# apache/tez

Measured on NVIDIA H100. Metric: sorted KV GB/s (16B key / 64B val), higher is better.
Workload: dtype u8

## Files before the change

tez_b200/csrc/common.cuh:

```cuda
#pragma once
#include <cuda_runtime.h>
#include <stdint.h>
#include <stdio.h>

#include <stdexcept>
#include <string>

namespace tezgpu {

struct Error : public std::runtime_error {
  int code;
  Error(int c, const std::string &m) : std::runtime_error(m), code(c) {}
};

#define TG_CUDA(expr)                                                                                   \
  do {                                                                                                  \
    cudaError_t _e = (expr);                                                                            \
    if (_e != cudaSuccess) {                                                                            \
      throw ::tezgpu::Error(_e == cudaErrorMemoryAllocation ? -3 : -2,                                  \
                            std::string(#expr) + ": " + cudaGetErrorString(_e) + " (" + __FILE__ + ":" + \
                                std::to_string(__LINE__) + ")");                                        \
    }                                                                                                   \
  } while (0)

#define TG_CHECK(cond, code, msg)                      \
  do {                                                 \
    if (!(cond)) throw ::tezgpu::Error((code), (msg)); \
  } while (0)

static inline uint64_t div_up(uint64_t a, uint64_t b) { return (a + b - 1) / b; }
static inline uint64_t align_up(uint64_t a, uint64_t b) { return div_up(a, b) * b; }

enum { CMP_BYTES = 0, CMP_TEXT = 1, CMP_BYTESWRITABLE = 2, CMP_INT = 3, CMP_LONG = 4 };

__host__ __device__ __forceinline__ int vint_decode_size(uint8_t first) {
  int v = (int)(int8_t)first;
  if (v >= -112) return 1;
  if (v < -120) return -119 - v;
  return -111 - v;
}
__host__ __device__ __forceinline__ int vint_size_u32(uint32_t v) {
  if (v <= 127) return 1;
  if (v < (1u << 8)) return 2;
  if (v < (1u << 16)) return 3;
  if (v < (1u << 24)) return 4;
  return 5;
}
__host__ __device__ __forceinline__ uint8_t vint_byte_u32(uint32_t v, int b) {
  int sz = vint_size_u32(v);
  if (sz == 1) return (uint8_t)v;
  if (b == 0) return (uint8_t)(-112 - (sz - 1));
  int shift = (sz - 1 - b) * 8;
  return (uint8_t)(v >> shift);
}

__device__ __forceinline__ uint32_t key_content_skip(int cmp, const uint8_t *key, uint32_t klen) {
  if (klen == 0) return 0;
  if (cmp == CMP_TEXT) {
    uint32_t s = (uint32_t)vint_decode_size(key[0]);
    return s < klen ? s : klen;
  }
  if (cmp == CMP_BYTESWRITABLE) return klen < 4 ? klen : 4;
  return 0;
}

__device__ __forceinline__ uint32_t norm_byte(int cmp, const uint8_t *content, uint32_t i) {
  uint32_t b = content[i];
  if (i == 0 && (cmp == CMP_INT || cmp == CMP_LONG)) b ^= 0x80u;
  return b;
}

__device__ __forceinline__ int32_t hash_bytes_dev(const uint8_t *p, uint32_t n) {
  uint32_t h = 1;
  for (uint32_t i = 0; i < n; i++) h = 31u * h + (uint32_t)(int32_t)(int8_t)p[i];
  return (int32_t)h;
}

__device__ __forceinline__ int32_t key_hash_dev(int cmp, const uint8_t *key, uint32_t klen) {
  if (cmp == CMP_INT && klen >= 4)
    return (int32_t)(((uint32_t)key[0] << 24) | ((uint32_t)key[1] << 16) | ((uint32_t)key[2] << 8) | key[3]);
  if (cmp == CMP_LONG && klen >= 8) {
    uint64_t v = 0;
    for (int i = 0; i < 8; i++) v = (v << 8) | key[i];
    return (int32_t)(uint32_t)(v ^ (v >> 32));
  }
  uint32_t s = key_content_skip(cmp, key, klen);
  return hash_bytes_dev(key + s, klen - s);
}

__device__ __forceinline__ uint32_t lanemask_lt() {
  uint32_t m;
  asm("mov.u32 %0, %%lanemask_lt;" : "=r"(m));
  return m;
}

__device__ __forceinline__ uint32_t ld_volatile_u32(const uint32_t *p) {
  uint32_t v;
  asm volatile("ld.volatile.global.u32 %0, [%1];" : "=r"(v) : "l"(p) : "memory");
  return v;
}
__device__ __forceinline__ void st_volatile_u32(uint32_t *p, uint32_t v) {
  asm volatile("st.volatile.global.u32 [%0], %1;" ::"l"(p), "r"(v) : "memory");
}

__device__ __forceinline__ uint64_t ld_volatile_u64(const uint64_t *p) {
  uint64_t v;
  asm volatile("ld.volatile.global.u64 %0, [%1];" : "=l"(v) : "l"(p) : "memory");
  return v;
}
__device__ __forceinline__ void st_volatile_u64(uint64_t *p, uint64_t v) {
  asm volatile("st.volatile.global.u64 [%0], %1;" ::"l"(p), "l"(v) : "memory");
}

}
```

tez_b200/csrc/radix_sort.cuh:

```cuda
#pragma once
#include "common.cuh"

#ifndef TEZGPU_RADIX_THREADS32
#define TEZGPU_RADIX_THREADS32 512
#endif
#ifndef TEZGPU_RADIX_IPT32
#define TEZGPU_RADIX_IPT32 16
#endif
#ifndef TEZGPU_RADIX_LOOKBACK
#define TEZGPU_RADIX_LOOKBACK 8
#endif
#ifndef TEZGPU_RANK_MODE
#define TEZGPU_RANK_MODE 2
#endif

namespace tezgpu {

constexpr int RADIX_BITS = 8;
constexpr int RADIX = 1 << RADIX_BITS;
constexpr uint32_t STATE_FLAG_LOCAL = 1u << 30;
constexpr uint32_t STATE_FLAG_INCL = 2u << 30;
constexpr uint32_t STATE_VALUE_MASK = (1u << 30) - 1;
constexpr uint32_t RADIX_MAX_N = (1u << 30) - 1;

template <typename KeyT>
__device__ __forceinline__ uint32_t radix_digit(KeyT k, int shift) {
  return (uint32_t)(k >> shift) & (RADIX - 1);
}

template <typename KeyT, int NPASS>
__global__ void __launch_bounds__(512) k_radix_hist(const KeyT *__restrict__ keys, uint32_t n, int begin_bit,
                                                    uint32_t *__restrict__ hist ) {
  __shared__ uint32_t s_hist[NPASS * RADIX];
  for (int i = threadIdx.x; i < NPASS * RADIX; i += blockDim.x) s_hist[i] = 0;
  __syncthreads();
  uint32_t stride = gridDim.x * blockDim.x;
  for (uint32_t i = blockIdx.x * blockDim.x + threadIdx.x; i < n; i += stride) {
    KeyT k = keys[i];
#pragma unroll
    for (int p = 0; p < NPASS; p++) atomicAdd(&s_hist[p * RADIX + radix_digit(k, begin_bit + p * RADIX_BITS)], 1u);
  }
  __syncthreads();
  for (int i = threadIdx.x; i < NPASS * RADIX; i += blockDim.x) {
    uint32_t c = s_hist[i];
    if (c) atomicAdd(&hist[i], c);
  }
}

__global__ void __launch_bounds__(RADIX) k_radix_scan_hist(uint32_t *__restrict__ hist, int npass, uint32_t n,
                                                          uint32_t *__restrict__ trivial) {
  __shared__ uint32_t s_warp[RADIX / 32];
  const int tid = threadIdx.x, lane = tid & 31, warp = tid >> 5;
  for (int p = 0; p < npass; p++) {
    uint32_t c = hist[p * RADIX + tid];
    uint32_t incl = c;
#pragma unroll
    for (int o = 1; o < 32; o <<= 1) {
      uint32_t t = __shfl_up_sync(0xffffffffu, incl, o);
      if (lane >= o) incl += t;
    }
    if (lane == 31) s_warp[warp] = incl;
    __syncthreads();
    uint32_t base = 0;
    for (int w = 0; w < warp; w++) base += s_warp[w];
    hist[p * RADIX + tid] = base + incl - c;
    uint32_t any = __syncthreads_or(c == n && n > 0);
    if (tid == 0 && trivial) trivial[p] = any ? 1u : 0u;
    __syncthreads();
  }
}

template <typename KeyT, int THREADS, int IPT>
struct OnesweepCfg {
  static constexpr int NWARPS = THREADS / 32;
  static constexpr int TILE = THREADS * IPT;
  static constexpr size_t SMEM = (size_t)TILE * (sizeof(KeyT) + sizeof(uint32_t)) + (size_t)NWARPS * RADIX * 4 +
                                 2 * RADIX * 4 + 64 + (TEZGPU_RANK_MODE == 2 ? (size_t)NWARPS * RADIX * 4 : 0);
};

template <typename KeyT, int THREADS, int IPT, bool VALS_IOTA>
__global__ void __launch_bounds__(THREADS, 1024 / THREADS)
    k_onesweep_pass(const KeyT *__restrict__ keys_in, KeyT *__restrict__ keys_out, const uint32_t *__restrict__ vals_in,
                    uint32_t *__restrict__ vals_out, uint32_t n, int shift, const uint32_t *__restrict__ hist_base,
                    uint32_t *tile_state, uint32_t *tile_counter) {
  using Cfg = OnesweepCfg<KeyT, THREADS, IPT>;
  constexpr int NWARPS = Cfg::NWARPS;
  constexpr int TILE = Cfg::TILE;
  static_assert(THREADS >= RADIX, "one thread per digit for the look-back");

  extern __shared__ __align__(16) uint8_t smem_raw[];
  KeyT *s_keys = reinterpret_cast<KeyT *>(smem_raw);
  uint32_t *s_vals = reinterpret_cast<uint32_t *>(smem_raw + (size_t)TILE * sizeof(KeyT));
  uint32_t *s_wcnt = s_vals + TILE;
  uint32_t *s_dstart = s_wcnt + NWARPS * RADIX;
  uint32_t *s_goff = s_dstart + RADIX;
  uint32_t *s_misc = s_goff + RADIX;
#if TEZGPU_RANK_MODE == 2
  uint32_t *s_wmask = s_misc + 16;
#endif

  const int tid = threadIdx.x, lane = tid & 31, warp = tid >> 5;

#ifdef TEZGPU_TICKET_ATOMIC
  if (tid == 0) s_misc[0] = atomicAdd(tile_counter, 1u);
#else
  if (tid == 0) s_misc[0] = blockIdx.x;
#endif
  for (int i = tid; i < NWARPS * RADIX; i += THREADS) s_wcnt[i] = 0;
#if TEZGPU_RANK_MODE == 2
  for (int i = tid; i < NWARPS * RADIX; i += THREADS) s_wmask[i] = 0;
#endif
  __syncthreads();
  const uint32_t tile = s_misc[0];
  const uint32_t tile_base = tile * (uint32_t)TILE;
  const uint32_t tile_n = min((uint32_t)TILE, n - tile_base);
  const uint32_t warp_base = (uint32_t)warp * 32u * IPT;

  KeyT key[IPT];
  uint32_t rnk[IPT];
#pragma unroll
  for (int j = 0; j < IPT; j++) {
    uint32_t li = warp_base + j * 32 + lane;
    key[j] = (li < tile_n) ? keys_in[tile_base + li] : (KeyT)0;
  }
  uint32_t *wc = s_wcnt + warp * RADIX;
  const uint32_t lt = lanemask_lt();
#pragma unroll
  for (int j = 0; j < IPT; j++) {
    uint32_t li = warp_base + j * 32 + lane;
    bool valid = li < tile_n;
    uint32_t d = radix_digit(key[j], shift);
    uint32_t peers;
#if TEZGPU_RANK_MODE == 0
    peers = __match_any_sync(0xffffffffu, valid ? d : (uint32_t)RADIX);
#elif TEZGPU_RANK_MODE == 2
    {
      uint32_t *wm = s_wmask + warp * RADIX;
      if (valid) atomicOr(&wm[d], 1u << lane);
      __syncwarp();
      peers = valid ? wm[d] : 0u;
      __syncwarp();
      if (valid) atomicAnd(&wm[d], ~(1u << lane));
    }
#else
    peers = __ballot_sync(0xffffffffu, valid);
    if (!valid) peers = ~peers;
#pragma unroll
    for (int b = 0; b < RADIX_BITS; b++) {
      const bool bit = (d >> b) & 1u;
      const uint32_t bm = __ballot_sync(0xffffffffu, bit);
      peers &= bit ? bm : ~bm;
    }
#endif
    uint32_t pre = 0;
    if (valid && (peers & lt) == 0) pre = atomicAdd(&wc[d], (uint32_t)__popc(peers));
    pre = __shfl_sync(0xffffffffu, pre, __ffs(peers) - 1);
    rnk[j] = pre + __popc(peers & lt);
  }
  __syncthreads();

  uint32_t count = 0;
  if (tid < RADIX) {
    uint32_t run = 0;
#pragma unroll
    for (int w = 0; w < NWARPS; w++) {
      uint32_t c = s_wcnt[w * RADIX + tid];
      s_wcnt[w * RADIX + tid] = run;
      run += c;
    }
    count = run;
    st_volatile_u32(&tile_state[(size_t)tile * RADIX + tid], (tile == 0 ? STATE_FLAG_INCL : STATE_FLAG_LOCAL) | count);
    uint32_t incl = count;
#pragma unroll
    for (int o = 1; o < 32; o <<= 1) {
      uint32_t t = __shfl_up_sync(0xffffffffu, incl, o);
      if (lane >= o) incl += t;
    }
    if (lane == 31) s_misc[1 + warp] = incl;
    s_dstart[tid] = incl - count;
  }
  __syncthreads();
  if (tid < RADIX) {
    uint32_t base = 0;
    for (int w = 0; w < warp; w++) base += s_misc[1 + w];
    s_dstart[tid] += base;
  }
  __syncthreads();

#pragma unroll
  for (int j = 0; j < IPT; j++) {
    uint32_t li = warp_base + j * 32 + lane;
    if (li < tile_n) {
      uint32_t d = radix_digit(key[j], shift);
      uint32_t slot = s_dstart[d] + wc[d] + rnk[j];
      s_keys[slot] = key[j];
      uint32_t v;
      if (VALS_IOTA) v = tile_base + li;
      else v = vals_in[tile_base + li];
      s_vals[slot] = v;
    }
  }

  if (tid < RADIX) {
    uint32_t excl = 0;
    if (tile > 0) {
      constexpr int LOOKBACK = TEZGPU_RADIX_LOOKBACK;
      int64_t t = (int64_t)tile - 1;
      bool done = false;
      while (!done) {
        uint32_t st[LOOKBACK];
#ifdef TEZGPU_RADIX_DEBUG
        if (tid == 0) atomicAdd(tile_counter + 7, 1u);
#endif
#pragma unroll
        for (int b = 0; b < LOOKBACK; b++)
          st[b] = (t - b >= 0) ? ld_volatile_u32(&tile_state[(size_t)(t - b) * RADIX + tid]) : STATE_FLAG_INCL;
#pragma unroll
        for (int b = 0; b < LOOKBACK; b++) {
          if (done) break;
          uint32_t flag = st[b] & ~STATE_VALUE_MASK;
          if (flag == 0) break;
          excl += st[b] & STATE_VALUE_MASK;
          t--;
          if (flag == STATE_FLAG_INCL) done = true;
        }
      }
      st_volatile_u32(&tile_state[(size_t)tile * RADIX + tid], STATE_FLAG_INCL | (excl + count));
    }
    s_goff[tid] = hist_base[tid] + excl - s_dstart[tid];
  }
  __syncthreads();

#pragma unroll
  for (int k = 0; k < IPT; k++) {
    uint32_t slot = (uint32_t)tid + k * THREADS;
    if (slot < tile_n) {
      KeyT kk = s_keys[slot];
      uint32_t dest = s_goff[radix_digit(kk, shift)] + slot;
      keys_out[dest] = kk;
      vals_out[dest] = s_vals[slot];
    }
  }
}

struct RadixWorkspace {
  uint32_t *hist = nullptr;
  uint32_t *trivial = nullptr;
  uint32_t *tile_state = nullptr;
  uint32_t *tile_counter = nullptr;
  size_t tile_state_words = 0;
};

template <typename KeyT>
struct RadixTuning {
  static constexpr int THREADS = sizeof(KeyT) == 4 ? TEZGPU_RADIX_THREADS32 : 512;
  static constexpr int IPT = sizeof(KeyT) == 4 ? TEZGPU_RADIX_IPT32 : 10;
};

template <typename KeyT>
static inline uint32_t radix_num_tiles(uint32_t n) {
  using T = RadixTuning<KeyT>;
  return (uint32_t)div_up(n, (uint64_t)T::THREADS * T::IPT);
}
template <typename KeyT>
static inline size_t radix_tile_state_words(uint32_t n, int npass) {
  return (size_t)radix_num_tiles<KeyT>(n) * RADIX * (size_t)npass;
}

template <typename KeyT>
static int radix_sort_passes(cudaStream_t st, const RadixWorkspace &ws, KeyT *keys_a, KeyT *keys_b, uint32_t *vals_a,
                             uint32_t *vals_b, uint32_t n, int begin_bit, int npass, uint32_t pass_mask,
                             bool first_vals_iota, int *launches) {
  using T = RadixTuning<KeyT>;
  using Cfg = OnesweepCfg<KeyT, T::THREADS, T::IPT>;
  static bool attr_set = false;
  if (!attr_set) {
    TG_CUDA(cudaFuncSetAttribute(k_onesweep_pass<KeyT, T::THREADS, T::IPT, false>,
                                 cudaFuncAttributeMaxDynamicSharedMemorySize, (int)Cfg::SMEM));
    TG_CUDA(cudaFuncSetAttribute(k_onesweep_pass<KeyT, T::THREADS, T::IPT, true>,
                                 cudaFuncAttributeMaxDynamicSharedMemorySize, (int)Cfg::SMEM));
    attr_set = true;
  }
  uint32_t ntiles = radix_num_tiles<KeyT>(n);
  TG_CHECK((size_t)ntiles * RADIX * (size_t)npass <= ws.tile_state_words, -1, "radix workspace too small");
  TG_CUDA(cudaMemsetAsync(ws.tile_state, 0, (size_t)ntiles * RADIX * (size_t)npass * 4, st));
  TG_CUDA(cudaMemsetAsync(ws.tile_counter, 0, 8 * 4, st));
  int done = 0;
  bool iota = first_vals_iota;
  for (int p = 0; p < npass; p++) {
    if (!((pass_mask >> p) & 1u)) continue;
    KeyT *kin = (done & 1) ? keys_b : keys_a, *kout = (done & 1) ? keys_a : keys_b;
    uint32_t *vin = (done & 1) ? vals_b : vals_a, *vout = (done & 1) ? vals_a : vals_b;
    uint32_t *state = ws.tile_state + (size_t)p * ntiles * RADIX;
    if (iota)
      k_onesweep_pass<KeyT, T::THREADS, T::IPT, true><<<ntiles, T::THREADS, Cfg::SMEM, st>>>(
          kin, kout, vin, vout, n, begin_bit + p * RADIX_BITS, ws.hist + p * RADIX, state, ws.tile_counter + p);
    else
      k_onesweep_pass<KeyT, T::THREADS, T::IPT, false><<<ntiles, T::THREADS, Cfg::SMEM, st>>>(
          kin, kout, vin, vout, n, begin_bit + p * RADIX_BITS, ws.hist + p * RADIX, state, ws.tile_counter + p);
    TG_CUDA(cudaGetLastError());
    if (launches) (*launches)++;
    iota = false;
    done++;
  }
  return done;
}

}
```

tez_b200/csrc/sorter.cuh:

```cuda
#pragma once
#include <stdlib.h>
#include <string.h>

#include <vector>

#include "../../include/tezgpu.h"
#include "device_util.h"
#ifndef TEZGPU_EMIT_ROUND_FILL_DEFAULT
#define TEZGPU_EMIT_ROUND_FILL_DEFAULT 0
#endif
#include "emit_pipe_u.cuh"
#include "emit_tma.cuh"
#include "emit_runs.cuh"
#include "sorter_kernels.cuh"

namespace tezgpu {

__global__ void k_store_to_host(uint32_t *__restrict__ dst0, const uint32_t *__restrict__ src0, uint32_t n0, uint32_t *__restrict__ dst1,
                                const uint32_t *__restrict__ src1, uint32_t n1, uint32_t *__restrict__ dst2,
                                const uint32_t *__restrict__ src2, uint32_t n2) {
  for (uint32_t i = threadIdx.x; i < n0; i += blockDim.x) dst0[i] = src0[i];
  for (uint32_t i = threadIdx.x; i < n1; i += blockDim.x) dst1[i] = src1[i];
  for (uint32_t i = threadIdx.x; i < n2; i += blockDim.x) dst2[i] = src2[i];
  __threadfence_system();
}
static inline void store_to_host(cudaStream_t st, void *d0, const void *s0, size_t b0, void *d1 = nullptr, const void *s1 = nullptr,
                                 size_t b1 = 0, void *d2 = nullptr, const void *s2 = nullptr, size_t b2 = 0) {
  k_store_to_host<<<1, 256, 0, st>>>((uint32_t *)d0, (const uint32_t *)s0, (uint32_t)(b0 / 4), (uint32_t *)d1, (const uint32_t *)s1,
                                     (uint32_t)(b1 / 4), (uint32_t *)d2, (const uint32_t *)s2, (uint32_t)(b2 / 4));
}


static inline int partition_bits(int P) {
  int b = 0;
  while ((1ll << b) < (long long)P) b++;
  return b;
}

struct DeviceConstants {
  CrcTables *d_crc = nullptr;
  static DeviceConstants &get(int device) {
    static DeviceConstants inst[64];
    DeviceConstants &d = inst[device & 63];
    if (!d.d_crc) {
      CrcTables *h = new CrcTables();
      crc_build_tables(*h, EMIT_CRC_STRIDE_WORDS);
      TG_CUDA(cudaMalloc((void **)&d.d_crc, sizeof(CrcTables)));
      TG_CUDA(cudaMemcpy(d.d_crc, h, sizeof(CrcTables), cudaMemcpyHostToDevice));
      delete h;
    }
    return d;
  }
};

struct FramingMismatch {};

class SortPipeline {
 public:
  tezgpu_conf conf;
  int pbits;
  cudaStream_t stream = nullptr;
  EventTimer timer;
  int num_sms = 132;

  DeviceBuffer keysA, keysB, valsA, valsB, same, blk, small, tile_state, sizes, rec_off;
  DeviceBuffer t_pos[2], t_gid[2], t_lidx[2], t_key64[2], t_val[2], t_state, t_ghead, t_gneq, sym_sets, sym_tab, rep_flags;
  DeviceBuffer seg_start, tile_start, part_start, d_index, seg_crc, tile_desc, tile_crc, tie_state;
  PinnedBuffer h_small;

  explicit SortPipeline(const tezgpu_conf &c) : conf(c) {
    TG_CHECK(c.num_partitions >= 1, TEZGPU_E_INVALID, "num_partitions must be >= 1");
    TG_CHECK(c.comparator >= TEZGPU_CMP_BYTES && c.comparator <= TEZGPU_CMP_LONG, TEZGPU_E_UNSUPPORTED,
             "comparator outside the device-supported set (BYTES, TEXT, BYTESWRITABLE, INT, LONG)");
    TG_CHECK(c.partitioner == TEZGPU_PART_GIVEN || c.partitioner == TEZGPU_PART_HASH, TEZGPU_E_UNSUPPORTED,
             "partitioner outside the device-supported set (GIVEN, HASH)");
    int ndev = 0;
    cudaError_t e = cudaGetDeviceCount(&ndev);
    if (e != cudaSuccess || ndev == 0) {
      cudaGetLastError();
      throw Error(TEZGPU_E_CUDA, "no CUDA device available (libtezgpu has no CPU fallback)");
    }
    TG_CHECK(c.device >= 0 && c.device < ndev, TEZGPU_E_INVALID, "bad device ordinal");
    TG_CUDA(cudaSetDevice(c.device));
    TG_CUDA(cudaStreamCreateWithFlags(&stream, cudaStreamNonBlocking));
    TG_CUDA(cudaDeviceGetAttribute(&num_sms, cudaDevAttrMultiProcessorCount, c.device));
    {
      const char *g = getenv("TEZGPU_L2_FETCH");
      int gran = g ? atoi(g) : 32;
      if (gran > 0 && cudaDeviceSetLimit(cudaLimitMaxL2FetchGranularity, (size_t)gran) != cudaSuccess) cudaGetLastError();
    }
    pbits = partition_bits(c.num_partitions);
    TG_CHECK(pbits <= 31, TEZGPU_E_INVALID, "too many partitions");
    h_small.ensure(4096);
    small.ensure(16384);
    DeviceConstants::get(c.device);
  }
  ~SortPipeline() {
    if (stream) cudaStreamDestroy(stream);
  }

  static uint64_t output_bound(uint64_t n, uint64_t kv_bytes, int P) { return kv_bytes + 12 * n + 10ull * P + 64; }

  uint32_t *d_hist() { return small.as<uint32_t>(); }
  uint32_t *d_trivial() { return small.as<uint32_t>() + 2048; }
  uint32_t *d_tile_counter() { return small.as<uint32_t>() + 2056; }
  int *d_error() { return reinterpret_cast<int *>(small.as<uint32_t>() + 2064); }
  uint32_t *d_large() { return small.as<uint32_t>() + 2065; }
  uint32_t *d_m() { return small.as<uint32_t>() + 2072; }
  unsigned long long *d_ties() { return reinterpret_cast<unsigned long long *>(small.as<uint32_t>() + 2074); }
  uint32_t *d_ticket() { return small.as<uint32_t>() + 2073; }
  unsigned long long *d_dups() { return reinterpret_cast<unsigned long long *>(small.as<uint32_t>() + 2066); }
  uint64_t *d_totals() { return reinterpret_cast<uint64_t *>(small.as<uint32_t>() + 2068); }

  struct SortState {
    Records rec;
    uint32_t *K = nullptr;
    uint32_t *order = nullptr;
    uint64_t dup_count = 0, tie_records = 0;
    int launches = 0;
    bool have_bounds = false, spec_layout = false;
    uint64_t spec_file_bytes = 0, spec_tiles = 0;
  } state;
  int merge_check_same = 1;
  bool merge_inputs_plain = false;
  uint32_t merge_max_runs = 0;
  static bool runs_emit_enabled() {
    static const bool on = getenv("TEZGPU_EMIT_RUNS") && atoi(getenv("TEZGPU_EMIT_RUNS")) != 0;
    return on;
  }

  EmitParams make_emit_params(const Records &rec, const uint32_t *order, int rle, bool merge_mode, uint8_t *d_out) {
    EmitParams e;
    memset(&e, 0, sizeof(e));
    e.rec = rec;
    e.order = order;
    e.same = same.as<uint8_t>();
    e.part_start = part_start.as<uint32_t>();
    e.seg_start = seg_start.as<uint64_t>();
    e.tile_start = tile_start.as<uint32_t>();
    e.out = d_out;
    e.seg_crc = seg_crc.as<uint32_t>();
    e.crc = DeviceConstants::get(conf.device).d_crc;
    e.rle = rle;
    e.send_empty = conf.send_empty_partition_details;
    e.unordered = conf.sorter_impl == TEZGPU_SORTER_UNORDERED;
    e.merge_mode = merge_mode ? 1 : 0;
    e.check_same = merge_check_same;
    e.P = conf.num_partitions;
    return e;
  }
  static bool pipe_unaligned_enabled() {
    static const bool on = !(getenv("TEZGPU_EMIT_PIPE_UNALIGNED") && atoi(getenv("TEZGPU_EMIT_PIPE_UNALIGNED")) == 0);
    return on;
  }
  void set_fixed_layout(EmitParams &e, const Records &rec) {
    int h = 0;
    for (int b = 0; b < vint_size_u32(rec.klen); b++) e.fixed_hdr[h++] = vint_byte_u32(rec.klen, b);
    for (int b = 0; b < vint_size_u32(rec.vlen); b++) e.fixed_hdr[h++] = vint_byte_u32(rec.vlen, b);
    e.fixed_hdr_len = h;
    e.rec_size = h + rec.klen + rec.vlen;
    e.recs_per_tile = std::max<uint32_t>(1, std::min<uint32_t>(EMIT_MAX_RECS, (FE_IMG_BYTES - 32) / e.rec_size));
    static const int round_fill = getenv("TEZGPU_EMIT_ROUND_FILL") ? atoi(getenv("TEZGPU_EMIT_ROUND_FILL")) : TEZGPU_EMIT_ROUND_FILL_DEFAULT;
    bool fill = round_fill != 0;
    const uint32_t stride = rec.klen + rec.vlen;
    const bool fast = stride >= 16 && stride % 16 == 0;
    const bool aligned = !rec.key_off && !rec.use_runs && (((uintptr_t)rec.kv & 15u) == 0);
    if (rec.use_runs && runs_emit_enabled() && emit_runs_fits(e.recs_per_tile, e.rec_size, merge_max_runs)) {
    } else if (fast && aligned && emit4_max_recs(e.rec_size) >= 1 && emit4_fits(emit4_max_recs(e.rec_size), stride / 16, e.rec_size)) {
      e.recs_per_tile = std::min<uint32_t>(e.recs_per_tile, emit4_max_recs(e.rec_size));
    } else if (pipe_unaligned_enabled()) {
      if (fast && !aligned && emit4u_max_recs(stride / 16) >= 32) {
        e.recs_per_tile = std::min<uint32_t>(e.recs_per_tile, emit4u_max_recs(stride / 16));
        fill = true;
      }
    }
    if (fill && e.recs_per_tile >= 32) {
      const uint32_t cap = e.recs_per_tile;
      uint32_t best = cap;
      double best_eff = 0;
      for (uint32_t r = cap; r >= cap - cap / 10; r--) {
        const uint64_t chunks = ((uint64_t)r * e.rec_size + 15 + 4 + 2 + 15) / 16;
        const uint64_t rounds = (chunks + FE_THREADS - 1) / FE_THREADS;
        const double eff = (double)r / (double)rounds;
        if (eff > best_eff) { best_eff = eff; best = r; }
      }
      e.recs_per_tile = best;
    }
    e.rec_off = nullptr;
  }

  void run(Records rec, uint8_t *d_out, uint64_t out_cap, uint64_t *out_len, int64_t *index, tezgpu_stats *stats) {
    sort_phase(rec);
    int rle;
    if (conf.rle_policy == TEZGPU_RLE_ON) rle = 1;
    else if (conf.rle_policy == TEZGPU_RLE_OFF) rle = 0;
    else rle = (conf.sorter_impl == 1) ? 0 : ((double)state.dup_count > 0.1 * (double)rec.n);
    if (conf.sorter_impl == TEZGPU_SORTER_UNORDERED) rle = 0;
    emit_phase(rle, false, d_out, out_cap, out_len, index, stats);
  }

  void sort_phase(Records rec) {
    TG_CUDA(cudaSetDevice(conf.device));
    const uint32_t n = rec.n;
    const int P = conf.num_partitions;
    TG_CHECK(n <= RADIX_MAX_N, TEZGPU_E_INVALID, "more than 2^30-1 records in one sort");
    rec.cmp = conf.comparator;
    rec.hash_partition = conf.partitioner == TEZGPU_PART_HASH;
    rec.num_partitions = P;
    rec.pbits = pbits;
    const bool unordered = conf.sorter_impl == TEZGPU_SORTER_UNORDERED;
    rec.unordered = unordered ? 1 : 0;
    TG_CHECK(rec.hash_partition || rec.partition || rec.use_runs || n == 0 || P == 1, TEZGPU_E_INVALID, "partition ids required (partitioner=GIVEN)");
    int launches = 0;
    state.have_bounds = state.spec_layout = false;
    timer.reset();
    timer.mark(stream);

    const size_t n4 = (size_t)(n ? n : 1) * 4;
    keysA.ensure(n4); keysB.ensure(n4); valsA.ensure(n4); valsB.ensure(n4);
    same.ensure(n ? n : 1);
    const uint32_t nblk = (uint32_t)div_up(n ? n : 1, SCAN_TILE);
    blk.ensure(((size_t)nblk + 2) * 8);
    part_start.ensure(((size_t)P + 1) * 4);
    seg_start.ensure(((size_t)P + 1) * 8);
    tile_start.ensure(((size_t)P + 1) * 4);
    d_index.ensure((size_t)P * 24);
    seg_crc.ensure((size_t)P * 4);
    h_small.ensure(4096 + (size_t)P * 24);

    TG_CUDA(cudaMemsetAsync(small.p, 0, 16384, stream));
    TG_CUDA(cudaMemsetAsync(seg_crc.p, 0, (size_t)P * 4, stream));

    uint64_t dup_count = 0;
    uint64_t tie_records = 0;
    uint32_t *K = keysA.as<uint32_t>();
    uint32_t *order = valsA.as<uint32_t>();

    uint32_t sym_npos = 0;
    if (n && !rec.fixed && !unordered && !(getenv("TEZGPU_NO_SYM") && atoi(getenv("TEZGPU_NO_SYM")))) {
      sym_sets.ensure(SYM_MAX_POS * 8 * 4);
      sym_tab.ensure(sizeof(SymTable));
      TG_CUDA(cudaMemsetAsync(sym_sets.p, 0, SYM_MAX_POS * 8 * 4, stream));
      k_symbols<<<(int)std::min<uint64_t>(div_up(n, 256), (uint64_t)num_sms * 8), 256, 0, stream>>>(rec, sym_sets.as<uint32_t>());
      launches++;
      uint32_t hs[SYM_MAX_POS * 8];
      TG_CUDA(cudaMemcpyAsync(hs, sym_sets.p, sizeof(hs), cudaMemcpyDeviceToHost, stream));
      TG_CUDA(cudaStreamSynchronize(stream));
      SymTable *t = new SymTable();
      memset(t, 0, sizeof(*t));
      const uint32_t avail = 32u - (uint32_t)pbits;
      uint32_t used = 0, np = 0;
      for (; np < (uint32_t)SYM_MAX_POS; np++) {
        uint32_t cnt = 0;
        for (int w = 0; w < 8; w++) cnt += (uint32_t)__builtin_popcount(hs[np * 8 + w]);
        if (cnt == 0) break;
        uint32_t bits = 0;
        while ((1u << bits) < cnt + 1) bits++;
        if (used + bits > avail) break;
        used += bits;
        t->shift[np] = (uint8_t)(avail - used);
        uint32_t rk = 0;
        for (uint32_t b = 0; b < 256; b++)
          if ((hs[np * 8 + (b >> 5)] >> (b & 31u)) & 1u) t->rank[np][b] = (uint8_t)(++rk);
      }
      t->npos = np;
      if (np > avail / 8) {
        TG_CUDA(cudaMemcpyAsync(sym_tab.p, t, sizeof(SymTable), cudaMemcpyHostToDevice, stream));
        TG_CUDA(cudaStreamSynchronize(stream));
        rec.sym = sym_tab.as<SymTable>();
        sym_npos = np;
      }
      delete t;
    }
    if (n) {
      TG_CUDA(cudaMemsetAsync(same.p, 0, n, stream));
      const bool fast16 = rec.fixed && !rec.key_off && !rec.use_runs && rec.klen == 16 && ((rec.klen + rec.vlen) % 16 == 0) && rec.cmp == CMP_BYTES &&
                          (((uintptr_t)rec.kv & 15u) == 0);
      int sgrid = (int)std::min<uint64_t>(div_up(n, 256), (uint64_t)num_sms * 16);
      if (fast16) k_stage<true><<<sgrid, 256, 0, stream>>>(rec, K, d_hist(), d_error());
      else k_stage<false><<<sgrid, 256, 0, stream>>>(rec, K, d_hist(), d_error());
      TG_CUDA(cudaGetLastError());
      k_radix_scan_hist<<<1, RADIX, 0, stream>>>(d_hist(), 4, n, d_trivial());
      TG_CUDA(cudaGetLastError());
      launches += 2;
      timer.mark(stream);

      RadixWorkspace ws;
      ws.hist = d_hist();
      ws.trivial = d_trivial();
      ws.tile_counter = d_tile_counter();
      ws.tile_state_words = radix_tile_state_words<uint32_t>(n, 4);
      tile_state.ensure(ws.tile_state_words * 4);
      ws.tile_state = tile_state.as<uint32_t>();
      uint32_t pass_mask = 0xF;
      if (unordered) {
        pass_mask = 0;
        for (int q = 0; q < 4; q++) if (8 * q + 8 > 32 - pbits) pass_mask |= 1u << q;
        if (!pass_mask) pass_mask = 1;
      }
      int done = radix_sort_passes<uint32_t>(stream, ws, keysA.as<uint32_t>(), keysB.as<uint32_t>(), valsA.as<uint32_t>(),
                                             valsB.as<uint32_t>(), n, 0, 4, pass_mask, true, &launches);
      if (done & 1) { K = keysB.as<uint32_t>(); order = valsB.as<uint32_t>(); }
      if (unordered) {
        k_flip_order<<<(uint32_t)div_up(n, 256), 256, 0, stream>>>(order, n);
        launches++;
      }
      timer.mark(stream);

      const uint32_t depth0 = rec.sym ? sym_npos : (uint32_t)((32 - pbits) / 8);
      int per_sm_tf = 0;
      TG_CUDA(cudaOccupancyMaxActiveBlocksPerMultiprocessor(&per_sm_tf, k_tie_fix, TIEFIX_THREADS, 0));
      if (!unordered)
        k_tie_fix<<<(uint32_t)std::min<uint64_t>(div_up(n, TIEFIX_TILE), (uint64_t)num_sms * std::max(per_sm_tf, 1)), TIEFIX_THREADS, 0, stream>>>(
            rec, K, order, n, depth0, same.as<uint8_t>(), d_dups(), d_large(), d_ties());
      const uint32_t *d_m_ptr = reinterpret_cast<const uint32_t *>(d_ties());
      k_part_bounds<<<(uint32_t)div_up((uint64_t)P + 1, 256), 256, 0, stream>>>(K, n, P, pbits, part_start.as<uint32_t>());
      launches += 2;
      state.have_bounds = true;
      state.spec_layout = false;
      if (rec.fixed) {
        EmitParams e = make_emit_params(rec, order, 0, false, nullptr);
        set_fixed_layout(e, rec);
        k_layout<<<1, 1024, 0, stream>>>(e, seg_start.as<uint64_t>(), tile_start.as<uint32_t>(), d_index.as<int64_t>(), d_totals());
        launches++;
        state.spec_layout = true;
      }
      TG_CUDA(cudaGetLastError());
      uint32_t *hw = h_small.as<uint32_t>();
      store_to_host(stream, hw, small.as<uint32_t>() + 2064, 32, hw + 8, d_m_ptr, 4, h_small.as<uint8_t>() + 4096, d_index.p,
                    state.spec_layout ? (size_t)P * 24 : 0);
      TG_CUDA(cudaGetLastError());
      TG_CUDA(cudaStreamSynchronize(stream));
      TG_CHECK(!(hw[0] & 1u), TEZGPU_E_INVALID, "Illegal partition (outside [0, numPartitions))");
      if (hw[0] & 2u) throw FramingMismatch();
      uint32_t m = hw[8];
      tie_records = m;
      memcpy(&dup_count, hw + 2, 8);
      memcpy(&state.spec_file_bytes, hw + 4, 8);
      memcpy(&state.spec_tiles, hw + 6, 8);
      uint64_t *hs = h_small.as<uint64_t>() + 16;
      if (hw[1]) {
        k_tie_count<<<nblk, SCAN_THREADS, 0, stream>>>(K, n, blk.as<uint64_t>());
        k_scan_block_sums<<<1, 1024, 0, stream>>>(blk.as<uint64_t>(), nblk);
        TG_CUDA(cudaMemcpyAsync(&hs[0], blk.as<uint64_t>() + nblk, 8, cudaMemcpyDeviceToHost, stream));
        TG_CUDA(cudaStreamSynchronize(stream));
        m = (uint32_t)hs[0];
        tie_records = m;
        for (int s2 = 0; s2 < 2; s2++) { t_pos[s2].ensure((size_t)m * 4); t_gid[s2].ensure((size_t)m * 4); t_lidx[s2].ensure((size_t)m * 4); }
        k_tie_compact<<<nblk, SCAN_THREADS, 0, stream>>>(K, order, n, blk.as<uint64_t>(), t_pos[0].as<uint32_t>(),
                                                         t_gid[0].as<uint32_t>(), t_lidx[0].as<uint32_t>());
        launches += 3;
        const uint32_t ngroups = (uint32_t)(hs[0] >> 32);
        int cur = 0;
        {
          t_ghead.ensure(((size_t)ngroups + 2) * 4);
          t_gneq.ensure((size_t)ngroups + 1);
          TG_CUDA(cudaMemsetAsync(t_gneq.p, 0, (size_t)ngroups + 1, stream));
          const uint32_t mgrid = (uint32_t)div_up(m, 256), mblk0 = (uint32_t)div_up(m, SCAN_TILE);
          k_group_heads<<<mgrid, 256, 0, stream>>>(t_gid[0].as<uint32_t>(), m, t_ghead.as<uint32_t>());
          k_group_equal<<<mgrid, 256, 0, stream>>>(rec, t_gid[0].as<uint32_t>(), t_lidx[0].as<uint32_t>(), t_ghead.as<uint32_t>(), m, depth0,
                                                 TIE_SMALL_MAX, t_gneq.as<uint8_t>());
          blk.ensure(((size_t)std::max(mblk0, nblk) + 2) * 8);
          k_group_mark<<<mblk0, SCAN_THREADS, 0, stream>>>(t_pos[0].as<uint32_t>(), t_gid[0].as<uint32_t>(), t_ghead.as<uint32_t>(),
                                                          t_gneq.as<uint8_t>(), m, TIE_SMALL_MAX, same.as<uint8_t>(), d_dups(), blk.as<uint64_t>());
          k_scan_block_sums<<<1, 1024, 0, stream>>>(blk.as<uint64_t>(), mblk0);
          launches += 4;
          TG_CUDA(cudaGetLastError());
          TG_CUDA(cudaMemcpyAsync(&hs[0], blk.as<uint64_t>() + mblk0, 8, cudaMemcpyDeviceToHost, stream));
          TG_CUDA(cudaStreamSynchronize(stream));
          const uint32_t m2 = (uint32_t)hs[0];
          if (m2) {
            k_group_compact<<<mblk0, SCAN_THREADS, 0, stream>>>(t_pos[0].as<uint32_t>(), t_gid[0].as<uint32_t>(), t_lidx[0].as<uint32_t>(),
                                                               t_ghead.as<uint32_t>(), t_gneq.as<uint8_t>(), m, TIE_SMALL_MAX, blk.as<uint64_t>(),
                                                               t_pos[1].as<uint32_t>(), t_gid[1].as<uint32_t>(), t_lidx[1].as<uint32_t>());
            launches++;
            TG_CUDA(cudaGetLastError());
            cur = 1;
          }
          m = m2;
        }
        uint32_t depth = depth0;
        while (m) {
          t_key64[0].ensure((size_t)m * 8); t_key64[1].ensure((size_t)m * 8); t_val[0].ensure((size_t)m * 4);
          const uint32_t mblk = (uint32_t)div_up(m, SCAN_TILE);
          k_ref_build_keys<<<(uint32_t)div_up(m, 256), 256, 0, stream>>>(rec, t_gid[cur].as<uint32_t>(), t_lidx[cur].as<uint32_t>(), m,
                                                                    depth, t_key64[0].as<uint64_t>());
          TG_CUDA(cudaMemsetAsync(d_hist(), 0, 8 * RADIX * 4, stream));
          k_radix_hist<uint64_t, 8><<<(int)std::min<uint64_t>(div_up(m, 512 * 8), (uint64_t)num_sms * 4), 512, 0, stream>>>(t_key64[0].as<uint64_t>(), m, 0, d_hist());
          k_radix_scan_hist<<<1, RADIX, 0, stream>>>(d_hist(), 8, m, d_trivial());
          launches += 3;
          TG_CUDA(cudaGetLastError());
          uint32_t *ht = h_small.as<uint32_t>() + 64;
          TG_CUDA(cudaMemcpyAsync(ht, d_trivial(), 8 * 4, cudaMemcpyDeviceToHost, stream));
          TG_CUDA(cudaStreamSynchronize(stream));
          uint32_t mask = 0;
          for (int q = 0; q < 8; q++) if (!ht[q]) mask |= 1u << q;
          RadixWorkspace w2 = ws;
          w2.tile_state_words = radix_tile_state_words<uint64_t>(m, 8);
          t_state.ensure(w2.tile_state_words * 4);
          w2.tile_state = t_state.as<uint32_t>();
          int d2 = radix_sort_passes<uint64_t>(stream, w2, t_key64[0].as<uint64_t>(), t_key64[1].as<uint64_t>(), t_lidx[cur].as<uint32_t>(),
                                               t_val[0].as<uint32_t>(), m, 0, 8, mask, false, &launches);
          const uint64_t *Ks = (d2 & 1) ? t_key64[1].as<uint64_t>() : t_key64[0].as<uint64_t>();
          const uint32_t *Ls = (d2 & 1) ? t_val[0].as<uint32_t>() : t_lidx[cur].as<uint32_t>();
          k_ref_apply_count<<<mblk, SCAN_THREADS, 0, stream>>>(Ks, Ls, t_pos[cur].as<uint32_t>(), m, order, same.as<uint8_t>(), d_dups(),
                                                              blk.as<uint64_t>());
          k_scan_block_sums<<<1, 1024, 0, stream>>>(blk.as<uint64_t>(), mblk);
          launches += 2;
          TG_CUDA(cudaMemcpyAsync(&hs[0], blk.as<uint64_t>() + mblk, 8, cudaMemcpyDeviceToHost, stream));
          TG_CUDA(cudaStreamSynchronize(stream));
          uint32_t m2 = (uint32_t)hs[0];
          if (m2) {
            k_ref_compact<<<mblk, SCAN_THREADS, 0, stream>>>(Ks, Ls, t_pos[cur].as<uint32_t>(), m, blk.as<uint64_t>(),
                                                            t_pos[cur ^ 1].as<uint32_t>(), t_gid[cur ^ 1].as<uint32_t>(),
                                                            t_lidx[cur ^ 1].as<uint32_t>());
            launches++;
            TG_CUDA(cudaGetLastError());
          }
          cur ^= 1;
          m = m2;
          depth += 3;
        }
        TG_CUDA(cudaMemcpyAsync(&hs[0], d_dups(), 8, cudaMemcpyDeviceToHost, stream));
        TG_CUDA(cudaStreamSynchronize(stream));
        dup_count = hs[0];
      }
    }
    timer.mark(stream);
    state.rec = rec;
    state.K = K;
    state.order = order;
    state.dup_count = dup_count;
    state.tie_records = tie_records;
    state.launches = launches;
  }

  void emit_phase(int rle, bool merge_mode, uint8_t *d_out, uint64_t out_cap, uint64_t *out_len, int64_t *index,
                  tezgpu_stats *stats) {
    TG_CUDA(cudaSetDevice(conf.device));
    TG_CHECK(((uintptr_t)d_out & 15u) == 0, TEZGPU_E_INVALID, "output buffer must be 16-byte aligned");
    const Records rec = state.rec;
    const uint32_t n = rec.n;
    const int P = conf.num_partitions;
    uint32_t *K = state.K, *order = state.order;
    const uint64_t dup_count = state.dup_count, tie_records = state.tie_records;
    int launches = state.launches;
    const CrcTables *d_crc = DeviceConstants::get(conf.device).d_crc;
    const size_t n4 = (size_t)(n ? n : 1) * 4;
    const uint32_t nblk = (uint32_t)div_up(n ? n : 1, SCAN_TILE);
    TG_CUDA(cudaMemsetAsync(seg_crc.p, 0, (size_t)P * 4, stream));
    if (timer.n > (n ? 4 : 2)) timer.n = n ? 4 : 2;

    EmitParams e = make_emit_params(rec, order, rle, merge_mode, d_out);
    if (!state.have_bounds) {
      k_part_bounds<<<(uint32_t)div_up((uint64_t)P + 1, 256), 256, 0, stream>>>(K, n, P, pbits, part_start.as<uint32_t>());
      launches++;
    }
    const bool no_repeats = !rle && (!merge_mode || (!merge_check_same && merge_inputs_plain));
    const bool fixed_emit = rec.fixed && (dup_count == 0 || no_repeats);
    uint64_t bound = output_bound(n, rec.fixed ? (uint64_t)n * (rec.klen + rec.vlen) : rec.kv_bytes, P);
    uint64_t *hs = h_small.as<uint64_t>();
    if (fixed_emit && state.spec_layout) {
      set_fixed_layout(e, rec);
      hs[0] = state.spec_file_bytes;
      hs[1] = state.spec_tiles;
    } else {
      if (fixed_emit) {
        set_fixed_layout(e, rec);
      } else {
        uint64_t avg = n ? (rec.fixed ? (uint64_t)(rec.klen + rec.vlen) : rec.kv_bytes / n) + 4 : 16;
        e.recs_per_tile = (uint32_t)std::max<uint64_t>(1, std::min<uint64_t>(EMIT_MAX_RECS, (EMIT_IMG_BYTES - 32) / avg));
        sizes.ensure(n4);
        rec_off.ensure(((size_t)n + 2) * 8);
        if (n) {
          rep_flags.ensure(n);
          k_emit_repeat_flags<<<(uint32_t)div_up(n, 256), 256, 0, stream>>>(e, K, rep_flags.as<uint8_t>());
          launches++;
          e.rep = rep_flags.as<uint8_t>();
          k_emit_sizes<<<(uint32_t)div_up(n, 256), 256, 0, stream>>>(e, K, sizes.as<uint32_t>());
          k_sum_u32_blocks<<<nblk, SCAN_THREADS, 0, stream>>>(sizes.as<uint32_t>(), n, blk.as<uint64_t>());
          k_scan_block_sums<<<1, 1024, 0, stream>>>(blk.as<uint64_t>(), nblk);
          k_scan_u32_apply<<<nblk, SCAN_THREADS, 0, stream>>>(sizes.as<uint32_t>(), n, blk.as<uint64_t>(), rec_off.as<uint64_t>());
          launches += 4;
          TG_CUDA(cudaGetLastError());
        } else {
// ... 138 lines not shown
```

Measured before the change: 481.4.

## Sort 32-bit radix keys as interleaved key/value pairs with relaxed look-back

The 32-bit onesweep radix sort now carries keys and indices as interleaved uint2 pairs between intermediate passes. Each element then moves with one 8-byte load and store instead of two separate 4-byte streams, and shared-memory staging is unified. Padding elements take a max key so the per-element validity checks in ranking and scatter can be dropped. It also switches look-back loads and stores from volatile to relaxed.gpu, and changes tuning to 384 threads with a look-back depth of 4. The buffers are merged so order lives at offset n inside the sort buffer, and the first pass's interleaved output risks less-coalesced writes.

Measured after the change: 502.2, median of 6. +4.3%, better.

```diff
diff --git a/tez_b200/csrc/common.cuh b/tez_b200/csrc/common.cuh
--- a/tez_b200/csrc/common.cuh
+++ b/tez_b200/csrc/common.cuh
@@ -94,13 +94,13 @@
   return m;
 }
 
-__device__ __forceinline__ uint32_t ld_volatile_u32(const uint32_t *p) {
+__device__ __forceinline__ uint32_t ld_relaxed_gpu_u32(const uint32_t *p) {
   uint32_t v;
-  asm volatile("ld.volatile.global.u32 %0, [%1];" : "=r"(v) : "l"(p) : "memory");
+  asm volatile("ld.relaxed.gpu.global.u32 %0, [%1];" : "=r"(v) : "l"(p) : "memory");
   return v;
 }
-__device__ __forceinline__ void st_volatile_u32(uint32_t *p, uint32_t v) {
-  asm volatile("st.volatile.global.u32 [%0], %1;" ::"l"(p), "r"(v) : "memory");
+__device__ __forceinline__ void st_relaxed_gpu_u32(uint32_t *p, uint32_t v) {
+  asm volatile("st.relaxed.gpu.global.u32 [%0], %1;" ::"l"(p), "r"(v) : "memory");
 }
 
 __device__ __forceinline__ uint64_t ld_volatile_u64(const uint64_t *p) {
diff --git a/tez_b200/csrc/radix_sort.cuh b/tez_b200/csrc/radix_sort.cuh
--- a/tez_b200/csrc/radix_sort.cuh
+++ b/tez_b200/csrc/radix_sort.cuh
@@ -2,13 +2,16 @@
 #include "common.cuh"
 
 #ifndef TEZGPU_RADIX_THREADS32
-#define TEZGPU_RADIX_THREADS32 512
+#define TEZGPU_RADIX_THREADS32 384
 #endif
 #ifndef TEZGPU_RADIX_IPT32
 #define TEZGPU_RADIX_IPT32 16
 #endif
+#ifndef TEZGPU_RADIX_MINB32
+#define TEZGPU_RADIX_MINB32 (1024 / TEZGPU_RADIX_THREADS32)
+#endif
 #ifndef TEZGPU_RADIX_LOOKBACK
-#define TEZGPU_RADIX_LOOKBACK 8
+#define TEZGPU_RADIX_LOOKBACK 4
 #endif
 #ifndef TEZGPU_RANK_MODE
 #define TEZGPU_RANK_MODE 2
@@ -70,6 +73,8 @@
   }
 }
 
+enum RadixIO : int { IO_SEP = 0, IO_SEP_IOTA = 1, IO_PAIR = 2 };
+
 template <typename KeyT, int THREADS, int IPT>
 struct OnesweepCfg {
   static constexpr int NWARPS = THREADS / 32;
@@ -78,17 +83,21 @@
                                  2 * RADIX * 4 + 64 + (TEZGPU_RANK_MODE == 2 ? (size_t)NWARPS * RADIX * 4 : 0);
 };
 
-template <typename KeyT, int THREADS, int IPT, bool VALS_IOTA>
-__global__ void __launch_bounds__(THREADS, 1024 / THREADS)
+template <typename KeyT, int THREADS, int IPT, int MINB, int IN, int OUT>
+__global__ void __launch_bounds__(THREADS, MINB)
     k_onesweep_pass(const KeyT *__restrict__ keys_in, KeyT *__restrict__ keys_out, const uint32_t *__restrict__ vals_in,
                     uint32_t *__restrict__ vals_out, uint32_t n, int shift, const uint32_t *__restrict__ hist_base,
                     uint32_t *tile_state, uint32_t *tile_counter) {
   using Cfg = OnesweepCfg<KeyT, THREADS, IPT>;
   constexpr int NWARPS = Cfg::NWARPS;
   constexpr int TILE = Cfg::TILE;
+  constexpr bool PAIRS = sizeof(KeyT) == 4;
   static_assert(THREADS >= RADIX, "one thread per digit for the look-back");
+  static_assert(PAIRS || (IN != IO_PAIR && OUT != IO_PAIR), "pairs carry 32-bit keys");
+  static_assert(OUT != IO_SEP_IOTA, "iota is an input layout");
 
   extern __shared__ __align__(16) uint8_t smem_raw[];
+  uint2 *s_pair = reinterpret_cast<uint2 *>(smem_raw);
   KeyT *s_keys = reinterpret_cast<KeyT *>(smem_raw);
   uint32_t *s_vals = reinterpret_cast<uint32_t *>(smem_raw + (size_t)TILE * sizeof(KeyT));
   uint32_t *s_wcnt = s_vals + TILE;
@@ -117,34 +126,41 @@
   const uint32_t warp_base = (uint32_t)warp * 32u * IPT;
 
   KeyT key[IPT];
+  uint32_t val[IN == IO_SEP_IOTA ? 1 : IPT];
   uint32_t rnk[IPT];
 #pragma unroll
   for (int j = 0; j < IPT; j++) {
-    uint32_t li = warp_base + j * 32 + lane;
-    key[j] = (li < tile_n) ? keys_in[tile_base + li] : (KeyT)0;
+    const uint32_t li = warp_base + j * 32 + lane;
+    const bool valid = li < tile_n;
+    if constexpr (IN == IO_PAIR) {
+      uint2 p = make_uint2(~0u, 0u);
+      if (valid) p = reinterpret_cast<const uint2 *>(keys_in)[tile_base + li];
+      key[j] = p.x;
+      val[j] = p.y;
+    } else {
+      key[j] = valid ? keys_in[tile_base + li] : ~(KeyT)0;
+      if constexpr (IN == IO_SEP) val[j] = valid ? vals_in[tile_base + li] : 0u;
+    }
   }
   uint32_t *wc = s_wcnt + warp * RADIX;
   const uint32_t lt = lanemask_lt();
 #pragma unroll
   for (int j = 0; j < IPT; j++) {
-    uint32_t li = warp_base + j * 32 + lane;
-    bool valid = li < tile_n;
-    uint32_t d = radix_digit(key[j], shift);
+    const uint32_t d = radix_digit(key[j], shift);
     uint32_t peers;
 #if TEZGPU_RANK_MODE == 0
-    peers = __match_any_sync(0xffffffffu, valid ? d : (uint32_t)RADIX);
+    peers = __match_any_sync(0xffffffffu, d);
 #elif TEZGPU_RANK_MODE == 2
     {
       uint32_t *wm = s_wmask + warp * RADIX;
-      if (valid) atomicOr(&wm[d], 1u << lane);
+      atomicOr(&wm[d], 1u << lane);
       __syncwarp();
-      peers = valid ? wm[d] : 0u;
+      peers = wm[d];
       __syncwarp();
-      if (valid) atomicAnd(&wm[d], ~(1u << lane));
+      atomicAnd(&wm[d], ~(1u << lane));
     }
 #else
-    peers = __ballot_sync(0xffffffffu, valid);
-    if (!valid) peers = ~peers;
+    peers = 0xffffffffu;
 #pragma unroll
     for (int b = 0; b < RADIX_BITS; b++) {
       const bool bit = (d >> b) & 1u;
@@ -153,7 +169,7 @@
     }
 #endif
     uint32_t pre = 0;
-    if (valid && (peers & lt) == 0) pre = atomicAdd(&wc[d], (uint32_t)__popc(peers));
+    if ((peers & lt) == 0) pre = atomicAdd(&wc[d], (uint32_t)__popc(peers));
     pre = __shfl_sync(0xffffffffu, pre, __ffs(peers) - 1);
     rnk[j] = pre + __popc(peers & lt);
   }
@@ -169,7 +185,7 @@
       run += c;
     }
     count = run;
-    st_volatile_u32(&tile_state[(size_t)tile * RADIX + tid], (tile == 0 ? STATE_FLAG_INCL : STATE_FLAG_LOCAL) | count);
+    st_relaxed_gpu_u32(&tile_state[(size_t)tile * RADIX + tid], (tile == 0 ? STATE_FLAG_INCL : STATE_FLAG_LOCAL) | count);
     uint32_t incl = count;
 #pragma unroll
     for (int o = 1; o < 32; o <<= 1) {
@@ -189,14 +205,15 @@
 
 #pragma unroll
   for (int j = 0; j < IPT; j++) {
-    uint32_t li = warp_base + j * 32 + lane;
-    if (li < tile_n) {
-      uint32_t d = radix_digit(key[j], shift);
-      uint32_t slot = s_dstart[d] + wc[d] + rnk[j];
+    const uint32_t d = radix_digit(key[j], shift);
+    const uint32_t slot = s_dstart[d] + wc[d] + rnk[j];
+    uint32_t v;
+    if constexpr (IN == IO_SEP_IOTA) v = tile_base + warp_base + j * 32 + lane;
+    else v = val[j];
+    if constexpr (PAIRS) {
+      s_pair[slot] = make_uint2((uint32_t)key[j], v);
+    } else {
       s_keys[slot] = key[j];
-      uint32_t v;
-      if (VALS_IOTA) v = tile_base + li;
-      else v = vals_in[tile_base + li];
       s_vals[slot] = v;
     }
   }
@@ -214,7 +231,7 @@
 #endif
 #pragma unroll
         for (int b = 0; b < LOOKBACK; b++)
-          st[b] = (t - b >= 0) ? ld_volatile_u32(&tile_state[(size_t)(t - b) * RADIX + tid]) : STATE_FLAG_INCL;
+          st[b] = (t - b >= 0) ? ld_relaxed_gpu_u32(&tile_state[(size_t)(t - b) * RADIX + tid]) : STATE_FLAG_INCL;
 #pragma unroll
         for (int b = 0; b < LOOKBACK; b++) {
           if (done) break;
@@ -225,7 +242,7 @@
           if (flag == STATE_FLAG_INCL) done = true;
         }
       }
-      st_volatile_u32(&tile_state[(size_t)tile * RADIX + tid], STATE_FLAG_INCL | (excl + count));
+      st_relaxed_gpu_u32(&tile_state[(size_t)tile * RADIX + tid], STATE_FLAG_INCL | (excl + count));
     }
     s_goff[tid] = hist_base[tid] + excl - s_dstart[tid];
   }
@@ -233,12 +250,25 @@
 
 #pragma unroll
   for (int k = 0; k < IPT; k++) {
-    uint32_t slot = (uint32_t)tid + k * THREADS;
+    const uint32_t slot = (uint32_t)tid + k * THREADS;
     if (slot < tile_n) {
-      KeyT kk = s_keys[slot];
-      uint32_t dest = s_goff[radix_digit(kk, shift)] + slot;
-      keys_out[dest] = kk;
-      vals_out[dest] = s_vals[slot];
+      KeyT kk;
+      uint32_t v;
+      if constexpr (PAIRS) {
+        const uint2 p = s_pair[slot];
+        kk = p.x;
+        v = p.y;
+      } else {
+        kk = s_keys[slot];
+        v = s_vals[slot];
+      }
+      const uint32_t dest = s_goff[radix_digit(kk, shift)] + slot;
+      if constexpr (OUT == IO_PAIR) {
+        reinterpret_cast<uint2 *>(keys_out)[dest] = make_uint2((uint32_t)kk, v);
+      } else {
+        keys_out[dest] = kk;
+        vals_out[dest] = v;
+      }
     }
   }
 }
@@ -255,6 +285,7 @@
 struct RadixTuning {
   static constexpr int THREADS = sizeof(KeyT) == 4 ? TEZGPU_RADIX_THREADS32 : 512;
   static constexpr int IPT = sizeof(KeyT) == 4 ? TEZGPU_RADIX_IPT32 : 10;
+  static constexpr int MINB = sizeof(KeyT) == 4 ? TEZGPU_RADIX_MINB32 : 2;
 };
 
 template <typename KeyT>
@@ -267,40 +298,73 @@
   return (size_t)radix_num_tiles<KeyT>(n) * RADIX * (size_t)npass;
 }
 
-template <typename KeyT>
-static int radix_sort_passes(cudaStream_t st, const RadixWorkspace &ws, KeyT *keys_a, KeyT *keys_b, uint32_t *vals_a,
-                             uint32_t *vals_b, uint32_t n, int begin_bit, int npass, uint32_t pass_mask,
-                             bool first_vals_iota, int *launches) {
+template <typename KeyT, int IN, int OUT>
+static void radix_launch_pass(cudaStream_t st, uint32_t ntiles, const KeyT *kin, KeyT *kout, const uint32_t *vin,
+                              uint32_t *vout, uint32_t n, int shift, const uint32_t *hist, uint32_t *state,
+                              uint32_t *counter) {
   using T = RadixTuning<KeyT>;
   using Cfg = OnesweepCfg<KeyT, T::THREADS, T::IPT>;
+  auto kern = k_onesweep_pass<KeyT, T::THREADS, T::IPT, T::MINB, IN, OUT>;
   static bool attr_set = false;
   if (!attr_set) {
-    TG_CUDA(cudaFuncSetAttribute(k_onesweep_pass<KeyT, T::THREADS, T::IPT, false>,
-                                 cudaFuncAttributeMaxDynamicSharedMemorySize, (int)Cfg::SMEM));
-    TG_CUDA(cudaFuncSetAttribute(k_onesweep_pass<KeyT, T::THREADS, T::IPT, true>,
-                                 cudaFuncAttributeMaxDynamicSharedMemorySize, (int)Cfg::SMEM));
+    TG_CUDA(cudaFuncSetAttribute(kern, cudaFuncAttributeMaxDynamicSharedMemorySize, (int)Cfg::SMEM));
     attr_set = true;
   }
-  uint32_t ntiles = radix_num_tiles<KeyT>(n);
+  kern<<<ntiles, T::THREADS, Cfg::SMEM, st>>>(kin, kout, vin, vout, n, shift, hist, state, counter);
+  TG_CUDA(cudaGetLastError());
+}
+
+template <typename KeyT>
+static uint32_t radix_prepare(cudaStream_t st, const RadixWorkspace &ws, uint32_t n, int npass) {
+  const uint32_t ntiles = radix_num_tiles<KeyT>(n);
   TG_CHECK((size_t)ntiles * RADIX * (size_t)npass <= ws.tile_state_words, -1, "radix workspace too small");
   TG_CUDA(cudaMemsetAsync(ws.tile_state, 0, (size_t)ntiles * RADIX * (size_t)npass * 4, st));
   TG_CUDA(cudaMemsetAsync(ws.tile_counter, 0, 8 * 4, st));
+  return ntiles;
+}
+
+
+static int radix_sort_pairs(cudaStream_t st, const RadixWorkspace &ws, uint32_t *blk_a, uint32_t *blk_b, uint32_t n,
+                            int begin_bit, int npass, uint32_t pass_mask, int *launches) {
+  const int total = __builtin_popcount(pass_mask & ((1u << npass) - 1));
+  TG_CHECK(total >= 1, -1, "radix sort without a pass");
+  const uint32_t ntiles = radix_prepare<uint32_t>(st, ws, n, npass);
   int done = 0;
-  bool iota = first_vals_iota;
+  for (int p = 0; p < npass; p++) {
+    if (!((pass_mask >> p) & 1u)) continue;
+    uint32_t *in = (done & 1) ? blk_b : blk_a, *out = (done & 1) ? blk_a : blk_b;
+    const bool first = done == 0, last = done + 1 == total;
+    const int shift = begin_bit + p * RADIX_BITS;
+    const uint32_t *hist = ws.hist + p * RADIX;
+    uint32_t *state = ws.tile_state + (size_t)p * ntiles * RADIX, *counter = ws.tile_counter + p;
+    if (first && last)
+      radix_launch_pass<uint32_t, IO_SEP_IOTA, IO_SEP>(st, ntiles, in, out, nullptr, out + n, n, shift, hist, state, counter);
+    else if (first)
+      radix_launch_pass<uint32_t, IO_SEP_IOTA, IO_PAIR>(st, ntiles, in, out, nullptr, nullptr, n, shift, hist, state, counter);
+    else if (last)
+      radix_launch_pass<uint32_t, IO_PAIR, IO_SEP>(st, ntiles, in, out, nullptr, out + n, n, shift, hist, state, counter);
+    else
+      radix_launch_pass<uint32_t, IO_PAIR, IO_PAIR>(st, ntiles, in, out, nullptr, nullptr, n, shift, hist, state, counter);
+    if (launches) (*launches)++;
+    done++;
+  }
+  return done;
+}
+
+template <typename KeyT>
+static int radix_sort_passes(cudaStream_t st, const RadixWorkspace &ws, KeyT *keys_a, KeyT *keys_b, uint32_t *vals_a,
+                             uint32_t *vals_b, uint32_t n, int begin_bit, int npass, uint32_t pass_mask, int *launches) {
+  static_assert(sizeof(KeyT) == 8, "32-bit keys are sorted as pairs (radix_sort_pairs)");
+  const uint32_t ntiles = radix_prepare<KeyT>(st, ws, n, npass);
+  int done = 0;
   for (int p = 0; p < npass; p++) {
     if (!((pass_mask >> p) & 1u)) continue;
     KeyT *kin = (done & 1) ? keys_b : keys_a, *kout = (done & 1) ? keys_a : keys_b;
     uint32_t *vin = (done & 1) ? vals_b : vals_a, *vout = (done & 1) ? vals_a : vals_b;
-    uint32_t *state = ws.tile_state + (size_t)p * ntiles * RADIX;
-    if (iota)
-      k_onesweep_pass<KeyT, T::THREADS, T::IPT, true><<<ntiles, T::THREADS, Cfg::SMEM, st>>>(
-          kin, kout, vin, vout, n, begin_bit + p * RADIX_BITS, ws.hist + p * RADIX, state, ws.tile_counter + p);
-    else
-      k_onesweep_pass<KeyT, T::THREADS, T::IPT, false><<<ntiles, T::THREADS, Cfg::SMEM, st>>>(
-          kin, kout, vin, vout, n, begin_bit + p * RADIX_BITS, ws.hist + p * RADIX, state, ws.tile_counter + p);
-    TG_CUDA(cudaGetLastError());
+    radix_launch_pass<KeyT, IO_SEP, IO_SEP>(st, ntiles, kin, kout, vin, vout, n, begin_bit + p * RADIX_BITS,
+                                            ws.hist + p * RADIX, ws.tile_state + (size_t)p * ntiles * RADIX,
+                                            ws.tile_counter + p);
     if (launches) (*launches)++;
-    iota = false;
     done++;
   }
   return done;
diff --git a/tez_b200/csrc/sorter.cuh b/tez_b200/csrc/sorter.cuh
--- a/tez_b200/csrc/sorter.cuh
+++ b/tez_b200/csrc/sorter.cuh
@@ -63,7 +63,7 @@
   EventTimer timer;
   int num_sms = 132;
 
-  DeviceBuffer keysA, keysB, valsA, valsB, same, blk, small, tile_state, sizes, rec_off;
+  DeviceBuffer sortA, sortB, same, blk, small, tile_state, sizes, rec_off;
   DeviceBuffer t_pos[2], t_gid[2], t_lidx[2], t_key64[2], t_val[2], t_state, t_ghead, t_gneq, sym_sets, sym_tab, rep_flags;
   DeviceBuffer seg_start, tile_start, part_start, d_index, seg_crc, tile_desc, tile_crc, tie_state;
   PinnedBuffer h_small;
@@ -217,7 +217,7 @@
     timer.mark(stream);
 
     const size_t n4 = (size_t)(n ? n : 1) * 4;
-    keysA.ensure(n4); keysB.ensure(n4); valsA.ensure(n4); valsB.ensure(n4);
+    sortA.ensure(2 * n4); sortB.ensure(2 * n4);
     same.ensure(n ? n : 1);
     const uint32_t nblk = (uint32_t)div_up(n ? n : 1, SCAN_TILE);
     blk.ensure(((size_t)nblk + 2) * 8);
@@ -233,8 +233,8 @@
 
     uint64_t dup_count = 0;
     uint64_t tie_records = 0;
-    uint32_t *K = keysA.as<uint32_t>();
-    uint32_t *order = valsA.as<uint32_t>();
+    uint32_t *K = sortA.as<uint32_t>();
+    uint32_t *order = sortA.as<uint32_t>() + n;
 
     uint32_t sym_npos = 0;
     if (n && !rec.fixed && !unordered && !(getenv("TEZGPU_NO_SYM") && atoi(getenv("TEZGPU_NO_SYM")))) {
@@ -298,9 +298,8 @@
         for (int q = 0; q < 4; q++) if (8 * q + 8 > 32 - pbits) pass_mask |= 1u << q;
         if (!pass_mask) pass_mask = 1;
       }
-      int done = radix_sort_passes<uint32_t>(stream, ws, keysA.as<uint32_t>(), keysB.as<uint32_t>(), valsA.as<uint32_t>(),
-                                             valsB.as<uint32_t>(), n, 0, 4, pass_mask, true, &launches);
-      if (done & 1) { K = keysB.as<uint32_t>(); order = valsB.as<uint32_t>(); }
+      int done = radix_sort_pairs(stream, ws, sortA.as<uint32_t>(), sortB.as<uint32_t>(), n, 0, 4, pass_mask, &launches);
+      if (done & 1) { K = sortB.as<uint32_t>(); order = sortB.as<uint32_t>() + n; }
       if (unordered) {
         k_flip_order<<<(uint32_t)div_up(n, 256), 256, 0, stream>>>(order, n);
         launches++;
@@ -400,7 +399,7 @@
           t_state.ensure(w2.tile_state_words * 4);
           w2.tile_state = t_state.as<uint32_t>();
           int d2 = radix_sort_passes<uint64_t>(stream, w2, t_key64[0].as<uint64_t>(), t_key64[1].as<uint64_t>(), t_lidx[cur].as<uint32_t>(),
-                                               t_val[0].as<uint32_t>(), m, 0, 8, mask, false, &launches);
+                                               t_val[0].as<uint32_t>(), m, 0, 8, mask, &launches);
           const uint64_t *Ks = (d2 & 1) ? t_key64[1].as<uint64_t>() : t_key64[0].as<uint64_t>();
           const uint32_t *Ls = (d2 & 1) ? t_val[0].as<uint32_t>() : t_lidx[cur].as<uint32_t>();
           k_ref_apply_count<<<mblk, SCAN_THREADS, 0, stream>>>(Ks, Ls, t_pos[cur].as<uint32_t>(), m, order, same.as<uint8_t>(), d_dups(),
```
